# pySTEPS/pysteps

Measured on NVIDIA H100. Metric: Mpix/s advected (2048^2 frame, 12 leadtimes), higher is better.
Workload: dtype f64 (trajectories, motion field, IDW); f32 precip in/out; u8/i16/f32 OpenCV-exact LK stages

## Files before the change

pysteps_b200/csrc/lk_features.cu:

```cuda
#include <math_constants.h>

#include "common.cuh"

namespace {

constexpr int TX = 32, TY = 8;

__global__ void __launch_bounds__(256)
masked_max_partial(const float *__restrict__ eig, const uint8_t *__restrict__ valid, size_t N,
                   float *__restrict__ part) {
    __shared__ float sm[8];
    float v = -CUDART_INF_F;
    const size_t stride = (size_t)gridDim.x * blockDim.x;
    for (size_t i = (size_t)blockIdx.x * blockDim.x + threadIdx.x; i < N; i += stride)
        if (!valid || valid[i]) v = fmaxf(v, eig[i]);
#pragma unroll
    for (int o = 16; o > 0; o >>= 1) v = fmaxf(v, __shfl_xor_sync(0xffffffffu, v, o));
    if ((threadIdx.x & 31) == 0) sm[threadIdx.x >> 5] = v;
    __syncthreads();
    if (threadIdx.x < 32) {
        v = threadIdx.x < 8 ? sm[threadIdx.x] : -CUDART_INF_F;
#pragma unroll
        for (int o = 4; o > 0; o >>= 1) v = fmaxf(v, __shfl_xor_sync(0xffffffffu, v, o));
        if (threadIdx.x == 0) part[blockIdx.x] = v;
    }
}

__global__ void __launch_bounds__(256)
masked_max_final(const float *__restrict__ part, int nparts, double quality, unsigned *__restrict__ state) {
    __shared__ float sm[8];
    float v = -CUDART_INF_F;
    for (int i = threadIdx.x; i < nparts; i += blockDim.x) v = fmaxf(v, part[i]);
#pragma unroll
    for (int o = 16; o > 0; o >>= 1) v = fmaxf(v, __shfl_xor_sync(0xffffffffu, v, o));
    if ((threadIdx.x & 31) == 0) sm[threadIdx.x >> 5] = v;
    __syncthreads();
    if (threadIdx.x == 0) {
        for (int i = 1; i < 8; i++) v = fmaxf(v, sm[i]);
        const double mx = (v == -CUDART_INF_F) ? 0.0 : (double)v;
        const float thr = (float)(mx * quality);
        state[0] = __float_as_uint(thr);
        state[1] = 0u;
        state[2] = (v == -CUDART_INF_F) ? 1u : 0u;
    }
}

__device__ __forceinline__ unsigned order_key(float v) {
    const unsigned u = __float_as_uint(v);
    return (u & 0x80000000u) ? ~u : (u | 0x80000000u);
}

__global__ void __launch_bounds__(TX *TY)
candidates_kernel(const float *__restrict__ eig, const uint8_t *__restrict__ valid, int h, int w,
                  unsigned *__restrict__ state, unsigned long long *__restrict__ keys, unsigned cap) {
    const int x = blockIdx.x * TX + threadIdx.x, y = blockIdx.y * TY + threadIdx.y;
    if (x < 1 || y < 1 || x >= w - 1 || y >= h - 1) return;
    const float thr = __uint_as_float(state[0]);
    const size_t i = (size_t)y * w + x;
    const float v = eig[i];
    if (!(v > thr) || v == 0.f) return;
    if (valid && !valid[i]) return;
    bool ismax = true;
#pragma unroll
    for (int dy = -1; dy <= 1; dy++)
#pragma unroll
        for (int dx = -1; dx <= 1; dx++) {
            float u = eig[(size_t)(y + dy) * w + (x + dx)];
            u = (u > thr) ? u : 0.f;
            ismax &= !(u > v);
        }
    if (!ismax) return;
    const unsigned slot = atomicAdd(&state[1], 1u);
    if (slot < cap) keys[slot] = ((unsigned long long)order_key(v) << 32) | (unsigned)i;
}

constexpr int SORT_BLOCK = 1024;
constexpr int SORT_TILE = 2 * SORT_BLOCK;

__device__ __forceinline__ void cmpswap_desc(unsigned long long &a, unsigned long long &b, bool desc) {
    if ((a < b) == desc) {
        const unsigned long long t = a; a = b; b = t;
    }
}

__global__ void __launch_bounds__(SORT_BLOCK)
bitonic_local_kernel(unsigned long long *__restrict__ keys, unsigned n, unsigned k_start, unsigned k_end) {
    __shared__ unsigned long long sm[SORT_TILE];
    const unsigned base = blockIdx.x * SORT_TILE;
    for (unsigned t = threadIdx.x; t < SORT_TILE; t += SORT_BLOCK) sm[t] = (base + t < n) ? keys[base + t] : 0ull;
    __syncthreads();
    for (unsigned k = k_start; k <= k_end; k <<= 1) {
        const unsigned jmax = (k_start == k_end && k_start > SORT_TILE) ? SORT_TILE / 2 : k / 2;
        for (unsigned j = (jmax < k / 2 ? jmax : k / 2); j > 0; j >>= 1) {
            const unsigned t = threadIdx.x;
            const unsigned lo = 2 * t - (t & (j - 1));
            const unsigned hi = lo + j;
            const bool desc = (((base + lo) & k) == 0);
            cmpswap_desc(sm[lo], sm[hi], desc);
            __syncthreads();
        }
    }
    for (unsigned t = threadIdx.x; t < SORT_TILE; t += SORT_BLOCK)
        if (base + t < n) keys[base + t] = sm[t];
}

__global__ void __launch_bounds__(256)
bitonic_global_kernel(unsigned long long *__restrict__ keys, unsigned n, unsigned k, unsigned j) {
    const unsigned t = blockIdx.x * blockDim.x + threadIdx.x;
    if (t >= n / 2) return;
    const unsigned lo = 2 * t - (t & (j - 1));
    const unsigned hi = lo + j;
    const bool desc = ((lo & k) == 0);
    unsigned long long a = keys[lo], b = keys[hi];
    if ((a < b) == desc) { keys[lo] = b; keys[hi] = a; }
}

constexpr int CELL_CAP = 8;

__device__ __forceinline__ bool too_close(float dx, float dy, double md2) {
    return (double)__fadd_rn(__fmul_rn(dx, dx), __fmul_rn(dy, dy)) < md2;
}

struct SelectParams {
    const unsigned long long *keys;
    const unsigned *state;
    unsigned cap;
    int h, w, max_corners;
    double md2;
    bool use_dist;
    int cell, gw, gh;
    int *cell_cnt;
    short2 *cell_pts;
    float *out_xy;
    int *out_count;
};

__global__ void __launch_bounds__(32) select_kernel(const SelectParams p) {
    const int lane = threadIdx.x;
    const unsigned ncand = min(p.state[1], p.cap);
    int accepted = 0;
    const bool limited = p.max_corners > 0;
    for (unsigned basei = 0; basei < ncand; basei += 32) {
        const unsigned ci = basei + lane;
        bool ok = ci < ncand;
        int x = 0, y = 0;
        if (ok) {
            const unsigned addr = (unsigned)(p.keys[ci] & 0xffffffffull);
            y = addr / p.w;
            x = addr - y * p.w;
        }
        const int xc = x / p.cell, yc = y / p.cell;
        if (ok && p.use_dist) {
            const int x1 = max(0, xc - 1), y1 = max(0, yc - 1);
            const int x2 = min(p.gw - 1, xc + 1), y2 = min(p.gh - 1, yc + 1);
            for (int yy = y1; yy <= y2 && ok; yy++)
                for (int xx = x1; xx <= x2 && ok; xx++) {
                    const int c = yy * p.gw + xx;
                    const int cnt = min(p.cell_cnt[c], CELL_CAP);
                    for (int q = 0; q < cnt; q++) {
                        const short2 pt = p.cell_pts[c * CELL_CAP + q];
                        if (too_close((float)(x - pt.x), (float)(y - pt.y), p.md2)) { ok = false; break; }
                    }
                }
        }
        for (int i = 0; i < 32; i++) {
            const bool oki = __shfl_sync(0xffffffffu, ok, i);
            const int xi = __shfl_sync(0xffffffffu, x, i), yi = __shfl_sync(0xffffffffu, y, i);
            if (oki && lane > i && ok && p.use_dist && too_close((float)(x - xi), (float)(y - yi), p.md2))
                ok = false;
        }
        const unsigned bal = __ballot_sync(0xffffffffu, ok);
        const int rank = __popc(bal & ((1u << lane) - 1u));
        const bool take = ok && (!limited || accepted + rank < p.max_corners);
        const int c = yc * p.gw + xc;
        int before = 0;
        for (int i = 0; i < 32; i++) {
            const int ci2 = __shfl_sync(0xffffffffu, c, i);
            const bool ti = __shfl_sync(0xffffffffu, take, i);
            if (ti && i < lane && ci2 == c) before++;
        }
        if (take) {
            const int o = accepted + rank;
            p.out_xy[2 * o] = (float)x;
            p.out_xy[2 * o + 1] = (float)y;
            if (p.use_dist) {
                const int slot = p.cell_cnt[c] + before;
                if (slot < CELL_CAP) p.cell_pts[c * CELL_CAP + slot] = make_short2((short)x, (short)y);
            }
        }
        __syncwarp();
        if (take && p.use_dist) atomicAdd(&p.cell_cnt[c], 1);
        __threadfence_block();
        __syncwarp();
        accepted += __popc(bal);
        if (limited && accepted >= p.max_corners) { accepted = p.max_corners; break; }
    }
    if (lane == 0) *p.out_count = accepted;
}

constexpr int SEL_WARPS = 8;
constexpr unsigned SEL_DONE = 0xffffffffu;

__global__ void __launch_bounds__(32 * SEL_WARPS) select_smem_kernel(const SelectParams p) {
    extern __shared__ unsigned cells[];
    const int lane = threadIdx.x & 31, warp = threadIdx.x >> 5;
    const int ncell = p.gw * p.gh;
    volatile unsigned *ctl = cells + ncell;
    for (int i = threadIdx.x; i < ncell + 2; i += 32 * SEL_WARPS) cells[i] = 0u;
    __syncthreads();
    const unsigned ncand = min(p.state[1], p.cap);
    const unsigned nbatch = (ncand + 31u) / 32u;
    const unsigned md2i = (unsigned)ceil(p.md2);
    const bool limited = p.max_corners > 0;
    for (unsigned b = warp; b < nbatch; b += SEL_WARPS) {
        const unsigned ci = b * 32u + lane;
        bool ok = ci < ncand;
        int x = 0, y = 0;
        if (ok) {
            const unsigned addr = (unsigned)(p.keys[ci] & 0xffffffffull);
            y = addr / p.w;
            x = addr - y * p.w;
        }
        const int xc = x / p.cell, yc = y / p.cell;
        unsigned close = 0u;
#pragma unroll 8
        for (int i = 0; i < 32; i++) {
            const int xi = __shfl_sync(0xffffffffu, x, i), yi = __shfl_sync(0xffffffffu, y, i);
            const int dx = x - xi, dy = y - yi;
            if (i < lane && (unsigned)(dx * dx) + (unsigned)(dy * dy) < md2i) close |= 1u << i;
        }
        int nidx[9];
#pragma unroll
        for (int k = 0; k < 9; k++) {
            const int xx = xc + k % 3 - 1, yy = yc + k / 3 - 1;
            nidx[k] = (ok && xx >= 0 && yy >= 0 && xx < p.gw && yy < p.gh) ? yy * p.gw + xx : -1;
        }
        unsigned tok;
        while ((tok = ctl[0]) != b && tok != SEL_DONE) {}
        if (tok == SEL_DONE) break;
        __syncwarp();
        int accepted = (int)ctl[1];
        unsigned wds[9], any = 0u;
#pragma unroll
        for (int k = 0; k < 9; k++) {
            wds[k] = nidx[k] >= 0 ? cells[nidx[k]] : 0u;
            any |= wds[k];
        }
        if (any) {
#pragma unroll
            for (int k = 0; k < 9; k++) {
                const unsigned wd = wds[k];
                const int cnt = wd & 3u;
                const int ox = (xc + k % 3 - 1) * p.cell, oy = (yc + k / 3 - 1) * p.cell;
                for (int q = 0; q < cnt; q++) {
                    const unsigned f = (wd >> (2 + 10 * q)) & 0x3ffu;
                    if (too_close((float)(x - (ox + (int)(f & 31u))), (float)(y - (oy + (int)(f >> 5))), p.md2))
                        ok = false;
                }
            }
        }
        const unsigned okmask = __ballot_sync(0xffffffffu, ok);
        close &= okmask;
        unsigned acc = __ballot_sync(0xffffffffu, ok && close == 0u);
        unsigned pend = okmask & ~acc;
        while (pend) {
            const int i = __ffs(pend) - 1;
            pend &= pend - 1;
            const bool oki = (__shfl_sync(0xffffffffu, close, i) & acc) == 0u;
            if (oki) acc |= 1u << i;
        }
        ok = (acc >> lane) & 1u;
        const unsigned bal = __ballot_sync(0xffffffffu, ok);
        const int rank = __popc(bal & ((1u << lane) - 1u));
        const bool take = ok && (!limited || accepted + rank < p.max_corners);
        if (take) {
            const int o = accepted + rank;
            p.out_xy[2 * o] = (float)x;
            p.out_xy[2 * o + 1] = (float)y;
        }
        const unsigned tmask = __ballot_sync(0xffffffffu, take);
        const int c = yc * p.gw + xc;
        if (take) {
            const unsigned grp = __match_any_sync(tmask, c);
            if (lane == __ffs(grp) - 1) {
                unsigned wd = cells[c];
                unsigned g = grp;
                while (g) {
                    const int j = __ffs(g) - 1;
                    g &= g - 1;
                    const int xj = __shfl_sync(grp, x, j), yj = __shfl_sync(grp, y, j);
                    const unsigned cnt = wd & 3u;
                    if (cnt < 3u) {
                        const unsigned f = (unsigned)(xj - xc * p.cell) | ((unsigned)(yj - yc * p.cell) << 5);
                        wd = (wd & ~3u) | (f << (2 + 10 * cnt)) | (cnt + 1u);
                    }
                }
                cells[c] = wd;
            } else {
                unsigned g = grp;
                while (g) {
                    const int j = __ffs(g) - 1;
                    g &= g - 1;
                    __shfl_sync(grp, x, j);
                    __shfl_sync(grp, y, j);
                }
            }
        }
        __syncwarp();
        accepted += __popc(bal);
        const bool full = limited && accepted >= p.max_corners;
        if (full) accepted = p.max_corners;
        __threadfence_block();
        if (lane == 0) {
            ctl[1] = (unsigned)accepted;
            __threadfence_block();
            ctl[0] = full ? SEL_DONE : b + 1u;
        }
        if (full) break;
    }
    __syncthreads();
    if (threadIdx.x == 0) *p.out_count = (int)ctl[1];
}

}

extern "C" int b200_good_features(const float *eig, const uint8_t *valid, int m, int n, int max_corners,
                                  double quality_level, double min_distance, float *out_xy,
                                  int *out_count, void *stream) {
    B200_REQUIRE(eig && out_xy && out_count && m >= 1 && n >= 1 && max_corners > 0, "bad arguments");
    B200_REQUIRE((int64_t)m * n < ((int64_t)1 << 31), "image too large");
    cudaStream_t s = (cudaStream_t)stream;
    const size_t N = (size_t)m * n;
    const int nparts = b200::num_sms() * 4;
    b200::Scratch part, state, keys, cellc, cellp;
    B200_CUDA(part.alloc(sizeof(float) * nparts, s));
    B200_CUDA(state.alloc(sizeof(unsigned) * 4, s));
    masked_max_partial<<<nparts, 256, 0, s>>>(eig, valid, N, (float *)part.p);
    B200_LAUNCH_CHECK();
    masked_max_final<<<1, 256, 0, s>>>((const float *)part.p, nparts, quality_level, (unsigned *)state.p);
    B200_LAUNCH_CHECK();
    const unsigned cap = (unsigned)N;
    size_t cap_pow2 = SORT_TILE;
    while (cap_pow2 < (size_t)cap) cap_pow2 <<= 1;
    B200_CUDA(keys.alloc(sizeof(unsigned long long) * cap_pow2, s));
    candidates_kernel<<<dim3(b200::ceil_div(n, TX), b200::ceil_div(m, TY)), dim3(TX, TY), 0, s>>>(
        eig, valid, m, n, (unsigned *)state.p, (unsigned long long *)keys.p, cap);
    B200_LAUNCH_CHECK();
    unsigned hstate[4];
    B200_CUDA(cudaMemcpyAsync(hstate, state.p, sizeof(hstate), cudaMemcpyDeviceToHost, s));
    B200_CUDA(cudaStreamSynchronize(s));
    unsigned ncand = hstate[1] < cap ? hstate[1] : cap;
    if (hstate[2]) ncand = 0;
    if (ncand == 0) {
        B200_CUDA(cudaMemsetAsync(out_count, 0, sizeof(int), s));
        return 0;
    }
    unsigned npow = SORT_TILE;
    while (npow < ncand) npow <<= 1;
    if (npow > ncand)
        B200_CUDA(cudaMemsetAsync((unsigned long long *)keys.p + ncand, 0,
                                  sizeof(unsigned long long) * (npow - ncand), s));
    unsigned long long *K = (unsigned long long *)keys.p;
    bitonic_local_kernel<<<npow / SORT_TILE, SORT_BLOCK, 0, s>>>(K, npow, 2, SORT_TILE);
    B200_LAUNCH_CHECK();
    for (unsigned k = 2 * SORT_TILE; k <= npow; k <<= 1) {
        for (unsigned j = k / 2; j >= SORT_TILE; j >>= 1) {
            bitonic_global_kernel<<<b200::ceil_div((int)(npow / 2), 256), 256, 0, s>>>(K, npow, k, j);
            B200_LAUNCH_CHECK();
        }
        bitonic_local_kernel<<<npow / SORT_TILE, SORT_BLOCK, 0, s>>>(K, npow, k, k);
        B200_LAUNCH_CHECK();
    }
    SelectParams sp;
    sp.keys = K;
    sp.state = (const unsigned *)state.p;
    sp.cap = ncand;
    sp.h = m; sp.w = n;
    sp.max_corners = max_corners;
    sp.md2 = min_distance * min_distance;
    sp.use_dist = min_distance >= 1.0;
    sp.cell = sp.use_dist ? (int)lrint(min_distance) : 1;
    sp.gw = (n + sp.cell - 1) / sp.cell;
    sp.gh = (m + sp.cell - 1) / sp.cell;
    const size_t ncell = (size_t)sp.gw * sp.gh;
    sp.out_xy = out_xy;
    sp.out_count = out_count;
    if (sp.use_dist && sp.cell <= 32 && ncell * sizeof(unsigned) <= 200 * 1024) {
        const size_t smem = (ncell + 2) * sizeof(unsigned);
        B200_CUDA(cudaFuncSetAttribute(select_smem_kernel, cudaFuncAttributeMaxDynamicSharedMemorySize, (int)smem));
        select_smem_kernel<<<1, 32 * SEL_WARPS, smem, s>>>(sp);
        B200_LAUNCH_CHECK();
        return 0;
    }
    B200_CUDA(cellc.alloc(sizeof(int) * ncell, s));
    B200_CUDA(cellp.alloc(sizeof(short2) * ncell * CELL_CAP, s));
    B200_CUDA(cudaMemsetAsync(cellc.p, 0, sizeof(int) * ncell, s));
    sp.cell_cnt = (int *)cellc.p;
    sp.cell_pts = (short2 *)cellp.p;
    sp.out_xy = out_xy;
    sp.out_count = out_count;
    select_kernel<<<1, 32, 0, s>>>(sp);
    B200_LAUNCH_CHECK();
    return 0;
}
```

Measured before the change: 20140.

## Replace full bitonic sort with histogram top-slice sort and remove host sync

```diff
diff --git a/pysteps_b200/csrc/lk_features.cu b/pysteps_b200/csrc/lk_features.cu
--- a/pysteps_b200/csrc/lk_features.cu
+++ b/pysteps_b200/csrc/lk_features.cu
@@ -1,17 +1,37 @@
 #include <math_constants.h>
 
+#include <algorithm>
+
 #include "common.cuh"
 
 namespace {
 
 constexpr int TX = 32, TY = 8;
+
+constexpr int HIST_BITS = 16;
+constexpr int HIST_BINS = 1 << HIST_BITS;
+constexpr int SORT_THREADS = 1024;
+constexpr unsigned SORT_TILE = 16384;
+constexpr unsigned SLICE_MIN = 1024;
+constexpr unsigned SLICE_PER_CORNER = 3;
+constexpr int COMPACT_UNROLL = 4;
+
+enum : int {
+    ST_THR = 0,
+    ST_COUNT = 1,
+    ST_EMPTY = 2,
+    ST_SLICE = 3,
+    ST_RERUN = 4,
+    ST_WORDS = 5
+};
 
 __global__ void __launch_bounds__(256)
 masked_max_partial(const float *__restrict__ eig, const uint8_t *__restrict__ valid, size_t N,
-                   float *__restrict__ part) {
+                   float *__restrict__ part, unsigned *__restrict__ hist, int nbins) {
     __shared__ float sm[8];
     float v = -CUDART_INF_F;
     const size_t stride = (size_t)gridDim.x * blockDim.x;
+    for (int i = blockIdx.x * blockDim.x + threadIdx.x; i < nbins; i += (int)stride) hist[i] = 0u;
     for (size_t i = (size_t)blockIdx.x * blockDim.x + threadIdx.x; i < N; i += stride)
         if (!valid || valid[i]) v = fmaxf(v, eig[i]);
 #pragma unroll
@@ -39,9 +59,9 @@
         for (int i = 1; i < 8; i++) v = fmaxf(v, sm[i]);
         const double mx = (v == -CUDART_INF_F) ? 0.0 : (double)v;
         const float thr = (float)(mx * quality);
-        state[0] = __float_as_uint(thr);
-        state[1] = 0u;
-        state[2] = (v == -CUDART_INF_F) ? 1u : 0u;
+        state[ST_THR] = __float_as_uint(thr);
+        state[ST_EMPTY] = (v == -CUDART_INF_F) ? 1u : 0u;
+        state[ST_COUNT] = state[ST_SLICE] = state[ST_RERUN] = 0u;
     }
 }
 
@@ -52,10 +72,12 @@
 
 __global__ void __launch_bounds__(TX *TY)
 candidates_kernel(const float *__restrict__ eig, const uint8_t *__restrict__ valid, int h, int w,
-                  unsigned *__restrict__ state, unsigned long long *__restrict__ keys, unsigned cap) {
+                  unsigned *__restrict__ state, unsigned long long *__restrict__ keys, unsigned cap,
+                  unsigned *__restrict__ hist) {
     const int x = blockIdx.x * TX + threadIdx.x, y = blockIdx.y * TY + threadIdx.y;
     if (x < 1 || y < 1 || x >= w - 1 || y >= h - 1) return;
-    const float thr = __uint_as_float(state[0]);
+    if (state[ST_EMPTY]) return;
+    const float thr = __uint_as_float(state[ST_THR]);
     const size_t i = (size_t)y * w + x;
     const float v = eig[i];
     if (!(v > thr) || v == 0.f) return;
@@ -70,12 +92,12 @@
             ismax &= !(u > v);
         }
     if (!ismax) return;
-    const unsigned slot = atomicAdd(&state[1], 1u);
-    if (slot < cap) keys[slot] = ((unsigned long long)order_key(v) << 32) | (unsigned)i;
-}
-
-constexpr int SORT_BLOCK = 1024;
-constexpr int SORT_TILE = 2 * SORT_BLOCK;
+    const unsigned slot = atomicAdd(&state[ST_COUNT], 1u);
+    if (slot < cap) {
+        keys[slot] = ((unsigned long long)order_key(v) << 32) | (unsigned)i;
+        atomicAdd(&hist[order_key(v) >> (32 - HIST_BITS)], 1u);
+    }
+}
 
 __device__ __forceinline__ void cmpswap_desc(unsigned long long &a, unsigned long long &b, bool desc) {
     if ((a < b) == desc) {
@@ -83,36 +105,174 @@
     }
 }
 
-__global__ void __launch_bounds__(SORT_BLOCK)
-bitonic_local_kernel(unsigned long long *__restrict__ keys, unsigned n, unsigned k_start, unsigned k_end) {
-    __shared__ unsigned long long sm[SORT_TILE];
-    const unsigned base = blockIdx.x * SORT_TILE;
-    for (unsigned t = threadIdx.x; t < SORT_TILE; t += SORT_BLOCK) sm[t] = (base + t < n) ? keys[base + t] : 0ull;
-    __syncthreads();
-    for (unsigned k = k_start; k <= k_end; k <<= 1) {
-        const unsigned jmax = (k_start == k_end && k_start > SORT_TILE) ? SORT_TILE / 2 : k / 2;
-        for (unsigned j = (jmax < k / 2 ? jmax : k / 2); j > 0; j >>= 1) {
-            const unsigned t = threadIdx.x;
-            const unsigned lo = 2 * t - (t & (j - 1));
-            const unsigned hi = lo + j;
-            const bool desc = (((base + lo) & k) == 0);
-            cmpswap_desc(sm[lo], sm[hi], desc);
+__device__ void bitonic_smem(unsigned long long *sm, unsigned len, unsigned base, unsigned k_lo, unsigned k_hi) {
+    for (unsigned k = k_lo; k <= k_hi; k <<= 1) {
+        for (unsigned j = (k < len ? k : len) / 2; j > 0; j >>= 1) {
+            for (unsigned t = threadIdx.x; t < len / 2; t += SORT_THREADS) {
+                const unsigned lo = 2 * t - (t & (j - 1));
+                cmpswap_desc(sm[lo], sm[lo + j], ((base + lo) & k) == 0);
+            }
             __syncthreads();
         }
     }
-    for (unsigned t = threadIdx.x; t < SORT_TILE; t += SORT_BLOCK)
-        if (base + t < n) keys[base + t] = sm[t];
-}
-
-__global__ void __launch_bounds__(256)
-bitonic_global_kernel(unsigned long long *__restrict__ keys, unsigned n, unsigned k, unsigned j) {
-    const unsigned t = blockIdx.x * blockDim.x + threadIdx.x;
-    if (t >= n / 2) return;
-    const unsigned lo = 2 * t - (t & (j - 1));
-    const unsigned hi = lo + j;
-    const bool desc = ((lo & k) == 0);
-    unsigned long long a = keys[lo], b = keys[hi];
-    if ((a < b) == desc) { keys[lo] = b; keys[hi] = a; }
+}
+
+__device__ void bitonic_warp(unsigned long long *sm, unsigned len, unsigned k_lo, unsigned k_hi) {
+    const unsigned lane = threadIdx.x & 31, warp = threadIdx.x >> 5;
+    for (unsigned blk = warp * 64; blk < len; blk += SORT_THREADS * 2) {
+        const unsigned g = blk + 2 * lane;
+        unsigned long long a = sm[g], c = sm[g + 1];
+        for (unsigned k = k_lo; k <= k_hi; k <<= 1) {
+            const bool desc = (g & k) == 0;
+            for (unsigned j = (k < 64 ? k : 64) / 2; j > 1; j >>= 1) {
+                const unsigned long long pa = __shfl_xor_sync(0xffffffffu, a, j / 2);
+                const unsigned long long pc = __shfl_xor_sync(0xffffffffu, c, j / 2);
+                const bool lo = (g & j) == 0;
+                const bool keep_max = lo == desc;
+                a = keep_max ? (a > pa ? a : pa) : (a < pa ? a : pa);
+                c = keep_max ? (c > pc ? c : pc) : (c < pc ? c : pc);
+            }
+            cmpswap_desc(a, c, desc);
+        }
+        sm[g] = a;
+        sm[g + 1] = c;
+    }
+    __syncthreads();
+}
+
+__device__ void slice_bin(const unsigned *__restrict__ hist, unsigned target, unsigned *s_bin, unsigned *s_nsel,
+                          unsigned *wsum) {
+    constexpr int PER = HIST_BINS / SORT_THREADS;
+    static_assert(PER == 64, "the bin search takes two bins a lane");
+    const int t = threadIdx.x, lane = t & 31, warp = t >> 5;
+    const unsigned top = HIST_BINS - PER * t;
+    const uint4 *h4 = reinterpret_cast<const uint4 *>(hist + (top - PER));
+    unsigned c = 0;
+#pragma unroll
+    for (int i = 0; i < PER / 4; i++) {
+        const uint4 q = h4[i];
+        c += q.x + q.y + q.z + q.w;
+    }
+    unsigned inc = c;
+#pragma unroll
+    for (int o = 1; o < 32; o <<= 1) {
+        const unsigned u = __shfl_up_sync(0xffffffffu, inc, o);
+        if (lane >= o) inc += u;
+    }
+    if (lane == 31) wsum[warp] = inc;
+    __syncthreads();
+    if (warp == 0) {
+        unsigned w = wsum[lane];
+#pragma unroll
+        for (int o = 1; o < 32; o <<= 1) {
+            const unsigned u = __shfl_up_sync(0xffffffffu, w, o);
+            if (lane >= o) w += u;
+        }
+        wsum[lane] = w;
+    }
+    __syncthreads();
+    inc += warp ? wsum[warp - 1] : 0u;
+    const unsigned cross = __ballot_sync(0xffffffffu, inc - c < target && inc >= target);
+    if (cross) {
+        const int src = __ffs(cross) - 1;
+        const unsigned b0 = __shfl_sync(0xffffffffu, top, src) - 1u - 2u * lane;
+        const unsigned h0 = hist[b0], h1 = hist[b0 - 1];
+        unsigned pair = h0 + h1;
+#pragma unroll
+        for (int o = 1; o < 32; o <<= 1) {
+            const unsigned u = __shfl_up_sync(0xffffffffu, pair, o);
+            if (lane >= o) pair += u;
+        }
+        const unsigned above = __shfl_sync(0xffffffffu, inc - c, src) + pair - (h0 + h1);
+        const unsigned hit = __ballot_sync(0xffffffffu, above + h0 + h1 >= target);
+        if (lane == __ffs(hit) - 1) {
+            const bool first = above + h0 >= target;
+            *s_bin = first ? b0 : b0 - 1u;
+            *s_nsel = first ? above + h0 : above + h0 + h1;
+        }
+    }
+    __syncthreads();
+}
+
+__global__ void __launch_bounds__(SORT_THREADS)
+top_sort_kernel(const unsigned long long *__restrict__ src, const unsigned *__restrict__ count, unsigned cap,
+                const unsigned *__restrict__ hist, unsigned target, unsigned long long *__restrict__ dst,
+                unsigned *__restrict__ nsel_out) {
+    extern __shared__ unsigned long long sm[];
+    __shared__ unsigned s_bin, s_nsel, s_pos, wsum[32];
+    const unsigned n = min(*count, cap);
+    if (n == 0 && !nsel_out) return;
+    if (threadIdx.x == 0) {
+        s_bin = 0u;
+        s_nsel = n;
+        s_pos = 0u;
+    }
+    __syncthreads();
+    if (hist && n > target) slice_bin(hist, target, &s_bin, &s_nsel, wsum);
+    const unsigned bin = s_bin, nsel = s_nsel;
+    if (threadIdx.x == 0 && nsel_out) *nsel_out = nsel;
+    if (nsel == 0) return;
+    const bool in_smem = nsel <= SORT_TILE;
+    unsigned long long *out = in_smem ? sm : dst;
+    const int lane = threadIdx.x & 31;
+    for (unsigned base = 0; base < n; base += SORT_THREADS * COMPACT_UNROLL) {
+        unsigned long long key[COMPACT_UNROLL];
+#pragma unroll
+        for (int u = 0; u < COMPACT_UNROLL; u++) {
+            const unsigned i = base + u * SORT_THREADS + threadIdx.x;
+            key[u] = i < n ? src[i] : 0ull;
+        }
+#pragma unroll
+        for (int u = 0; u < COMPACT_UNROLL; u++) {
+            const unsigned i = base + u * SORT_THREADS + threadIdx.x;
+            const bool take = i < n && (unsigned)(key[u] >> (64 - HIST_BITS)) >= bin;
+            const unsigned bal = __ballot_sync(0xffffffffu, take);
+            unsigned pos = 0u;
+            if (lane == 0 && bal) pos = atomicAdd(&s_pos, (unsigned)__popc(bal));
+            pos = __shfl_sync(0xffffffffu, pos, 0);
+            if (take) out[pos + __popc(bal & ((1u << lane) - 1u))] = key[u];
+        }
+    }
+    unsigned npow = 1;
+    while (npow < nsel) npow <<= 1;
+    for (unsigned i = nsel + threadIdx.x; i < npow; i += SORT_THREADS) out[i] = 0ull;
+    __syncthreads();
+    if (in_smem) {
+        if (npow < 64) {
+            bitonic_smem(sm, npow, 0, 2, npow);
+        } else {
+            bitonic_warp(sm, npow, 2, 64);
+            for (unsigned k = 128; k <= npow; k <<= 1) {
+                for (unsigned j = k / 2; j >= 64; j >>= 1) {
+                    for (unsigned t = threadIdx.x; t < npow / 2; t += SORT_THREADS) {
+                        const unsigned lo = 2 * t - (t & (j - 1));
+                        cmpswap_desc(sm[lo], sm[lo + j], (lo & k) == 0);
+                    }
+                    __syncthreads();
+                }
+                bitonic_warp(sm, npow, k, k);
+            }
+        }
+        for (unsigned i = threadIdx.x; i < nsel; i += SORT_THREADS) dst[i] = sm[i];
+        return;
+    }
+    for (unsigned k = SORT_TILE; k <= npow; k <<= 1) {
+        for (unsigned j = k / 2; j >= SORT_TILE; j >>= 1) {
+            for (unsigned t = threadIdx.x; t < npow / 2; t += SORT_THREADS) {
+                const unsigned lo = 2 * t - (t & (j - 1));
+                unsigned long long a = dst[lo], b = dst[lo + j];
+                if ((a < b) == ((lo & k) == 0)) { dst[lo] = b; dst[lo + j] = a; }
+            }
+            __syncthreads();
+        }
+        for (unsigned base = 0; base < npow; base += SORT_TILE) {
+            for (unsigned i = threadIdx.x; i < SORT_TILE; i += SORT_THREADS) sm[i] = dst[base + i];
+            __syncthreads();
+            bitonic_smem(sm, SORT_TILE, base, k == SORT_TILE ? 2 : k, k);
+            for (unsigned i = threadIdx.x; i < SORT_TILE; i += SORT_THREADS) dst[base + i] = sm[i];
+            __syncthreads();
+        }
+    }
 }
 
 constexpr int CELL_CAP = 8;
@@ -123,8 +283,10 @@
 
 struct SelectParams {
     const unsigned long long *keys;
-    const unsigned *state;
+    const unsigned *count;
+    const unsigned *ncand;
     unsigned cap;
+    unsigned *rerun;
     int h, w, max_corners;
     double md2;
     bool use_dist;
@@ -135,9 +297,20 @@
     int *out_count;
 };
 
+__device__ __forceinline__ bool skip_rerun(const SelectParams &p) { return !p.ncand && *p.count == 0u; }
+
+__device__ __forceinline__ void finish_select(const SelectParams &p, unsigned nkeys, int accepted) {
+    *p.out_count = accepted;
+    if (p.ncand && accepted < p.max_corners) {
+        const unsigned ncand = min(*p.ncand, p.cap);
+        if (nkeys < ncand) *p.rerun = ncand;
+    }
+}
+
 __global__ void __launch_bounds__(32) select_kernel(const SelectParams p) {
+    if (skip_rerun(p)) return;
     const int lane = threadIdx.x;
-    const unsigned ncand = min(p.state[1], p.cap);
+    const unsigned ncand = *p.count;
     int accepted = 0;
     const bool limited = p.max_corners > 0;
     for (unsigned basei = 0; basei < ncand; basei += 32) {
@@ -195,20 +368,21 @@
         accepted += __popc(bal);
         if (limited && accepted >= p.max_corners) { accepted = p.max_corners; break; }
     }
-    if (lane == 0) *p.out_count = accepted;
+    if (lane == 0) finish_select(p, ncand, accepted);
 }
 
 constexpr int SEL_WARPS = 8;
 constexpr unsigned SEL_DONE = 0xffffffffu;
 
 __global__ void __launch_bounds__(32 * SEL_WARPS) select_smem_kernel(const SelectParams p) {
+    if (skip_rerun(p)) return;
     extern __shared__ unsigned cells[];
     const int lane = threadIdx.x & 31, warp = threadIdx.x >> 5;
     const int ncell = p.gw * p.gh;
     volatile unsigned *ctl = cells + ncell;
     for (int i = threadIdx.x; i < ncell + 2; i += 32 * SEL_WARPS) cells[i] = 0u;
     __syncthreads();
-    const unsigned ncand = min(p.state[1], p.cap);
+    const unsigned ncand = *p.count;
     const unsigned nbatch = (ncand + 31u) / 32u;
     const unsigned md2i = (unsigned)ceil(p.md2);
     const bool limited = p.max_corners > 0;
@@ -319,7 +493,7 @@
         if (full) break;
     }
     __syncthreads();
-    if (threadIdx.x == 0) *p.out_count = (int)ctl[1];
+    if (threadIdx.x == 0) finish_select(p, ncand, (int)ctl[1]);
 }
 
 }
@@ -332,49 +506,38 @@
     cudaStream_t s = (cudaStream_t)stream;
     const size_t N = (size_t)m * n;
     const int nparts = b200::num_sms() * 4;
-    b200::Scratch part, state, keys, cellc, cellp;
+    b200::Scratch part, state, hist, keys, order, cellc, cellp;
     B200_CUDA(part.alloc(sizeof(float) * nparts, s));
-    B200_CUDA(state.alloc(sizeof(unsigned) * 4, s));
-    masked_max_partial<<<nparts, 256, 0, s>>>(eig, valid, N, (float *)part.p);
-    B200_LAUNCH_CHECK();
-    masked_max_final<<<1, 256, 0, s>>>((const float *)part.p, nparts, quality_level, (unsigned *)state.p);
+    B200_CUDA(state.alloc(sizeof(unsigned) * ST_WORDS, s));
+    B200_CUDA(hist.alloc(sizeof(unsigned) * HIST_BINS, s));
+    unsigned *st = (unsigned *)state.p;
+    masked_max_partial<<<nparts, 256, 0, s>>>(eig, valid, N, (float *)part.p, (unsigned *)hist.p, HIST_BINS);
+    B200_LAUNCH_CHECK();
+    masked_max_final<<<1, 256, 0, s>>>((const float *)part.p, nparts, quality_level, st);
     B200_LAUNCH_CHECK();
     const unsigned cap = (unsigned)N;
     size_t cap_pow2 = SORT_TILE;
     while (cap_pow2 < (size_t)cap) cap_pow2 <<= 1;
-    B200_CUDA(keys.alloc(sizeof(unsigned long long) * cap_pow2, s));
+    B200_CUDA(keys.alloc(sizeof(unsigned long long) * cap, s));
+    B200_CUDA(order.alloc(sizeof(unsigned long long) * cap_pow2, s));
+    unsigned long long *K = (unsigned long long *)keys.p, *O = (unsigned long long *)order.p;
     candidates_kernel<<<dim3(b200::ceil_div(n, TX), b200::ceil_div(m, TY)), dim3(TX, TY), 0, s>>>(
-        eig, valid, m, n, (unsigned *)state.p, (unsigned long long *)keys.p, cap);
-    B200_LAUNCH_CHECK();
-    unsigned hstate[4];
-    B200_CUDA(cudaMemcpyAsync(hstate, state.p, sizeof(hstate), cudaMemcpyDeviceToHost, s));
-    B200_CUDA(cudaStreamSynchronize(s));
-    unsigned ncand = hstate[1] < cap ? hstate[1] : cap;
-    if (hstate[2]) ncand = 0;
-    if (ncand == 0) {
-        B200_CUDA(cudaMemsetAsync(out_count, 0, sizeof(int), s));
-        return 0;
-    }
-    unsigned npow = SORT_TILE;
-    while (npow < ncand) npow <<= 1;
-    if (npow > ncand)
-        B200_CUDA(cudaMemsetAsync((unsigned long long *)keys.p + ncand, 0,
-                                  sizeof(unsigned long long) * (npow - ncand), s));
-    unsigned long long *K = (unsigned long long *)keys.p;
-    bitonic_local_kernel<<<npow / SORT_TILE, SORT_BLOCK, 0, s>>>(K, npow, 2, SORT_TILE);
-    B200_LAUNCH_CHECK();
-    for (unsigned k = 2 * SORT_TILE; k <= npow; k <<= 1) {
-        for (unsigned j = k / 2; j >= SORT_TILE; j >>= 1) {
-            bitonic_global_kernel<<<b200::ceil_div((int)(npow / 2), 256), 256, 0, s>>>(K, npow, k, j);
-            B200_LAUNCH_CHECK();
-        }
-        bitonic_local_kernel<<<npow / SORT_TILE, SORT_BLOCK, 0, s>>>(K, npow, k, k);
-        B200_LAUNCH_CHECK();
-    }
+        eig, valid, m, n, st, K, cap, (unsigned *)hist.p);
+    B200_LAUNCH_CHECK();
+    const size_t sort_smem = sizeof(unsigned long long) * SORT_TILE;
+    B200_CUDA(cudaFuncSetAttribute(top_sort_kernel, cudaFuncAttributeMaxDynamicSharedMemorySize, (int)sort_smem));
+    const unsigned target = (unsigned)std::min<uint64_t>(
+        std::max<uint64_t>(SLICE_MIN, (uint64_t)SLICE_PER_CORNER * (uint64_t)max_corners), cap);
+    top_sort_kernel<<<1, SORT_THREADS, sort_smem, s>>>(K, st + ST_COUNT, cap, (const unsigned *)hist.p, target, O,
+                                                       st + ST_SLICE);
+    B200_LAUNCH_CHECK();
+
     SelectParams sp;
-    sp.keys = K;
-    sp.state = (const unsigned *)state.p;
-    sp.cap = ncand;
+    sp.keys = O;
+    sp.count = st + ST_SLICE;
+    sp.ncand = st + ST_COUNT;
+    sp.cap = cap;
+    sp.rerun = st + ST_RERUN;
     sp.h = m; sp.w = n;
     sp.max_corners = max_corners;
     sp.md2 = min_distance * min_distance;
@@ -383,23 +546,37 @@
     sp.gw = (n + sp.cell - 1) / sp.cell;
     sp.gh = (m + sp.cell - 1) / sp.cell;
     const size_t ncell = (size_t)sp.gw * sp.gh;
+    sp.cell_cnt = nullptr;
+    sp.cell_pts = nullptr;
     sp.out_xy = out_xy;
     sp.out_count = out_count;
-    if (sp.use_dist && sp.cell <= 32 && ncell * sizeof(unsigned) <= 200 * 1024) {
-        const size_t smem = (ncell + 2) * sizeof(unsigned);
-        B200_CUDA(cudaFuncSetAttribute(select_smem_kernel, cudaFuncAttributeMaxDynamicSharedMemorySize, (int)smem));
-        select_smem_kernel<<<1, 32 * SEL_WARPS, smem, s>>>(sp);
-        B200_LAUNCH_CHECK();
-        return 0;
-    }
-    B200_CUDA(cellc.alloc(sizeof(int) * ncell, s));
-    B200_CUDA(cellp.alloc(sizeof(short2) * ncell * CELL_CAP, s));
-    B200_CUDA(cudaMemsetAsync(cellc.p, 0, sizeof(int) * ncell, s));
-    sp.cell_cnt = (int *)cellc.p;
-    sp.cell_pts = (short2 *)cellp.p;
-    sp.out_xy = out_xy;
-    sp.out_count = out_count;
-    select_kernel<<<1, 32, 0, s>>>(sp);
+    SelectParams rp = sp;
+    rp.count = st + ST_RERUN;
+    rp.ncand = nullptr;
+    const bool smem_grid = sp.use_dist && sp.cell <= 32 && ncell * sizeof(unsigned) <= 200 * 1024;
+    const size_t sel_smem = (ncell + 2) * sizeof(unsigned);
+    if (smem_grid) {
+        B200_CUDA(cudaFuncSetAttribute(select_smem_kernel, cudaFuncAttributeMaxDynamicSharedMemorySize, (int)sel_smem));
+    } else {
+        B200_CUDA(cellc.alloc(sizeof(int) * ncell * 2, s));
+        B200_CUDA(cellp.alloc(sizeof(short2) * ncell * CELL_CAP * 2, s));
+        B200_CUDA(cudaMemsetAsync(cellc.p, 0, sizeof(int) * ncell * 2, s));
+        sp.cell_cnt = (int *)cellc.p;
+        sp.cell_pts = (short2 *)cellp.p;
+        rp.cell_cnt = sp.cell_cnt + ncell;
+        rp.cell_pts = sp.cell_pts + ncell * CELL_CAP;
+    }
+    if (smem_grid)
+        select_smem_kernel<<<1, 32 * SEL_WARPS, sel_smem, s>>>(sp);
+    else
+        select_kernel<<<1, 32, 0, s>>>(sp);
+    B200_LAUNCH_CHECK();
+    top_sort_kernel<<<1, SORT_THREADS, sort_smem, s>>>(K, st + ST_RERUN, cap, nullptr, 0u, O, nullptr);
+    B200_LAUNCH_CHECK();
+    if (smem_grid)
+        select_smem_kernel<<<1, 32 * SEL_WARPS, sel_smem, s>>>(rp);
+    else
+        select_kernel<<<1, 32, 0, s>>>(rp);
     B200_LAUNCH_CHECK();
     return 0;
 }
```

New measurement: 20180, median of 6. No clear change (+0.2%).
